# wuer5/OMGSR

Hardware: AMD Instinct MI355X
Metric: SR images/sec (higher is better)
Workload: dtype fp16; 1 GPU; OMGSR-S 256->1024, batch=4/GPU, accurate tier (fp32 stream, fp16 MFMA operands + split corrections), tiled VAE 256/64; global_batch=4, latent_tile=64, tile_overlap=32, world_size=1, parallelism=dp1, weights=seeded random, SD2.1-base shapes

## Files before the change

### omgsr_amd/build.py

```python
from __future__ import annotations

import hashlib
import os
import shutil
import subprocess
import sys

HERE = os.path.dirname(os.path.abspath(__file__))
CSRC = os.path.join(HERE, "csrc")
LIBDIR = os.path.join(HERE, "lib")
LIBNAME = "libomgsr_hip.so"
SOURCES = ["igemm.hip", "igemm_dma.hip", "igemm_p8.hip", "igemm_gmx.hip", "igemm_halo.hip", "igemm_halo_f16.hip", "igemm_halo_multi.hip", "igemm_halo_mx.hip", "igemm_halo_mx6.hip", "igemm_halo_mx6_flat.hip", "igemm_halo_out6.hip", "igemm_halo_flat.hip", "igemm_halo_gn.hip", "attention.hip", "norm.hip", "elementwise.hip", "colorfix.hip", "preprocess.hip", "mfma_peak.hip", "gemm_mxfp8.hip", "attention_mxfp8.hip"]
ARCH = "gfx950"


def lib_path() -> str:
    return os.path.join(LIBDIR, LIBNAME)


def _source_digest() -> str:
    h = hashlib.sha256()
    names = sorted(os.listdir(CSRC)) + [os.path.join("..", "..", "include", "omgsr_hip.h")]
    for n in names:
        p = os.path.join(CSRC, n)
        if os.path.isfile(p):
            h.update(n.encode())
            with open(p, "rb") as f:
                h.update(f.read())
    return h.hexdigest()


def build_library(force: bool = False, verbose: bool = False) -> str:
    hipcc = shutil.which("hipcc") or "/opt/rocm/bin/hipcc"
    os.makedirs(LIBDIR, exist_ok=True)
    out = lib_path()
    stamp = out + ".sha256"
    defs = ["-DOMGSR_BUILD_ABLATIONS"] if os.environ.get("OMGSR_BUILD_ABLATIONS", "0") == "1" else []
    defs += os.environ.get("OMGSR_EXTRA_DEFS", "").split()
    digest = _source_digest() + "".join(defs)
    if not force and os.path.isfile(out) and os.path.isfile(stamp) and open(stamp).read().strip() == digest:
        return out
    if not os.path.exists(hipcc):
        raise RuntimeError("hipcc not found: cannot build libomgsr_hip.so")
    from concurrent.futures import ThreadPoolExecutor

    hdr = hashlib.sha256()
    for n in sorted(os.listdir(CSRC)) + [os.path.join("..", "..", "include", "omgsr_hip.h")]:
        if n.endswith(".h"):
            with open(os.path.join(CSRC, n), "rb") as f:
                hdr.update(n.encode() + f.read())

    def compile_one(src: str) -> str:
        obj = os.path.join(LIBDIR, src.replace(".hip", ".o"))
        with open(os.path.join(CSRC, src), "rb") as f:
            want = hashlib.sha256(hdr.digest() + f.read() + "".join(defs).encode()).hexdigest()
        if not force and os.path.isfile(obj) and os.path.isfile(obj + ".sha256") and open(obj + ".sha256").read().strip() == want:
            return obj
        cmd = [hipcc, f"--offload-arch={ARCH}", "-O3", "-std=c++17", "-fPIC", "-Wall", "-Wno-unused-function", *defs,
               "-Rpass-analysis=kernel-resource-usage", "-c", os.path.join(CSRC, src), "-o", obj]
        if verbose:
            print(" ".join(cmd), file=sys.stderr)
        r = subprocess.run(cmd, stderr=subprocess.PIPE, text=True)
        import re
        remarks = [ln for ln in r.stderr.splitlines() if "remark:" in ln]
        rest, lines = [], r.stderr.splitlines()
        in_remark = False
        for i, ln in enumerate(lines):
            if "remark:" in ln:
                in_remark = True
                continue
            is_excerpt = bool(re.match(r"^\s*\d*\s*\|", ln)) or not ln.strip()
            if in_remark and is_excerpt:
                continue
            in_remark = False
            if ln.startswith("In file included from") and i + 1 < len(lines) and ("remark:" in lines[i + 1] or lines[i + 1].startswith("In file included")):
                continue
            if re.match(r"^\d+ (warning|remark)s? generated", ln):
                continue
            rest.append(ln)
        if rest:
            print("\n".join(rest), file=sys.stderr)
        if r.returncode != 0:
            raise subprocess.CalledProcessError(r.returncode, cmd)
        with open(os.path.join(LIBDIR, src + ".resources.txt"), "w") as f:
            f.write("\n".join(remarks) + "\n")
        with open(obj + ".sha256", "w") as f:
            f.write(want)
        return obj

    with ThreadPoolExecutor(max_workers=min(len(SOURCES), os.cpu_count() or 1)) as pool:
        objs = list(pool.map(compile_one, SOURCES))
    cmd = [hipcc, f"--offload-arch={ARCH}", "-shared", "-fPIC", "-o", out] + objs
    if verbose:
        print(" ".join(cmd), file=sys.stderr)
    subprocess.run(cmd, check=True)
    with open(stamp, "w") as f:
        f.write(digest)
    return out


def _short_name(mangled: str) -> str:
    import re
    m = re.match(r"_ZN12_GLOBAL__N_1(\d+)", mangled)
    if m:
        n = int(m.group(1))
        rest = mangled[m.end():]
        name, rest = rest[:n], rest[n:]
    else:
        m = re.match(r"_Z(\d+)", mangled)
        if not m:
            return mangled
        n = int(m.group(1))
        name, rest = mangled[m.end():m.end() + n], mangled[m.end() + n:]
    args = []
    if rest.startswith("I"):
        body = rest[1:]
        while body and not body.startswith("E"):
            for rx, fn in ((r"DF16_", lambda g: "fp16"), (r"DF16b", lambda g: "bf16"), (r"Lin(\d+)E", lambda g: "-" + g.group(1)),
                           (r"Li(\d+)E", lambda g: g.group(1)), (r"Lb([01])E", lambda g: g.group(1)), (r"f", lambda g: "float")):
                g = re.match(rx, body)
                if g:
                    args.append(fn(g))
                    body = body[g.end():]
                    break
            else:
                args.append("?")
                break
    return name + ("<" + ",".join(args) + ">" if args else "")


def kernel_resources() -> dict:
    import re
    build_library()
    keys = {"VGPRs": "vgpr", "AGPRs": "agpr", "SGPRs": "sgpr", "VGPRs Spill": "spill_vgpr", "SGPRs Spill": "spill_sgpr",
            "ScratchSize [bytes/lane]": "scratch", "Occupancy [waves/SIMD]": "occupancy", "LDS Size [bytes/block]": "lds"}
    out, mangled = {}, []
    for src in SOURCES:
        path = os.path.join(LIBDIR, src + ".resources.txt")
        if not os.path.isfile(path):
            build_library(force=True)
        cur = None
        for line in open(path):
            m = re.search(r"remark: (?:[^:]+:\d+:\d+: +)?([A-Za-z \[\]/]+): +(\S+)", line)
            if not m:
                continue
            k, v = m.group(1).strip(), m.group(2)
            if k == "Function Name":
                cur = {"source": src}
                mangled.append((v, cur))
            elif cur is not None and k in keys:
                cur[keys[k]] = int(v)
    for m, rec in mangled:
        k = _short_name(m)
        if "?" in k or k in out:
            k = m
        out[k] = rec
    return out


if __name__ == "__main__":
    print(build_library(force="--force" in sys.argv, verbose=True))
```

### omgsr_amd/csrc/igemm.hip

```cpp
#include "common.hip.h"
#include "../../include/omgsr_hip.h"
#include "timing.hip.h"
#include "igemm_epilogue.hip.h"
#include <stdlib.h>
#include <stdio.h>
#include <string.h>

namespace omgsr {
int igemm_dma_launch(const omgsr_igemm_args& a, IgemmGeo g, hipStream_t st);
int igemm_halo_launch(const omgsr_igemm_args& a, IgemmGeo g, hipStream_t st, bool phase = false);
int igemm_halo_launch_multi(const omgsr_igemm_args* a, const IgemmGeo* g0, int count, hipStream_t st, bool phase);
int igemm_halo_launch_splitk(const omgsr_igemm_args& a, const IgemmGeo& g0, int splits, hipStream_t st);
bool igemm_p8_wanted(const omgsr_igemm_args& a, const IgemmGeo& g);
int igemm_p8_launch(const omgsr_igemm_args& a, IgemmGeo g, hipStream_t st);
bool igemm_gmx_ok(const omgsr_igemm_args& a);
int igemm_gmx_launch(const omgsr_igemm_args& a, IgemmGeo g, hipStream_t st);
bool mxfp8_gemm_ok(const omgsr_igemm_args& a);
int mxfp8_gemm_launch(const omgsr_igemm_args& a, IgemmGeo g, hipStream_t st);
int igemm_halo_tiles(const omgsr_igemm_args& a, bool phase = false);
bool igemm_halo_out6_ok(const omgsr_igemm_args& a);
int igemm_halo_flat(const omgsr_igemm_args& a);
int igemm_halo_tiles_form(const omgsr_igemm_args& a, int flat);
int igemm_halo_gn_slots(const omgsr_igemm_args& a, bool phase = false);
bool igemm_halo_gn_geometry_ok(const omgsr_igemm_args& a);
}

namespace omgsr { static int g_batch_invariant = 0; }
extern "C" int omgsr_set_batch_invariant(int on) { omgsr::g_batch_invariant = (on != 0); return 0; }

namespace {

omgsr_igemm_args policy_view(const omgsr_igemm_args& a) {
    omgsr_igemm_args p = a;
    if (omgsr::g_batch_invariant && a.batch == 1) {
        const int64_t howo = (int64_t)a.Ho * a.Wo;
        const int64_t rows = a.sample_rows > 0 ? a.sample_rows : howo;
        if (rows >= howo) p.N = (int32_t)(rows / howo);
        else { p.N = 1; p.Ho = 1; p.Wo = (int32_t)rows; }
        if (p.N < 1) p.N = 1;
    }
    return p;
}

constexpr int BK = 32;
constexpr int ROWB = 80;
constexpr int NTHREADS = 256;

using Geo = IgemmGeo;

template <typename T, int BM, int BN, int WGM, int WGN>
__global__ __launch_bounds__(NTHREADS) void igemm_kernel(const omgsr_igemm_args p, const Geo g) {
    constexpr int WTM = BM / WGM, WTN = BN / WGN;
    constexpr int FM = WTM / 32, FN = WTN / 32;
    constexpr int A_CH = BM / 64, B_CH = BN / 64;
    static_assert(WGM * WGN == 4, "4 waves");
    static_assert(FM >= 1 && FN >= 1 && A_CH >= 1, "tile");
    constexpr int B_CHN = (B_CH >= 1) ? B_CH : 1;
    constexpr int STAGE_BYTES = (BM + BN) * ROWB;
    constexpr int EPI_BYTES = 4 * 32 * (WTN + 4) * 4;
    constexpr int LDS_BYTES = (2 * STAGE_BYTES > EPI_BYTES) ? 2 * STAGE_BYTES : EPI_BYTES;
    __shared__ __attribute__((aligned(16))) unsigned char lds[LDS_BYTES];

    const int t = threadIdx.x;
    const int lane = t & 63, wave = t >> 6;
    const int wm = wave / WGN, wn = wave % WGN;

    const int tile = xcd_remap(blockIdx.x, g.ntm * g.ntn);
    const int tn = tile % g.ntn, tm = tile / g.ntn;
    const int m0 = tm * BM, n0 = tn * BN;
    const int bz = blockIdx.z;

    const T* __restrict__ in = (const T*)p.in + (int64_t)bz * p.in_bstride;
    const T* __restrict__ wt = (const T*)p.weight + (int64_t)bz * p.w_bstride;

    const int kc = t & 3;
    const int r0 = t >> 2;
    int a_img[A_CH], a_vy0[A_CH], a_vx0[A_CH];
#pragma unroll
    for (int i = 0; i < A_CH; ++i) {
        const int m = m0 + r0 + 64 * i;
        if (m < g.M) {
            const int img = m / g.HoWo;
            const int rem = m - img * g.HoWo;
            const int oy = rem / p.Wo, ox = rem - oy * p.Wo;
            a_img[i] = img;
            a_vy0[i] = oy * p.stride - p.pad_top;
            a_vx0[i] = ox * p.stride - p.pad_left;
        } else {
            a_img[i] = -1; a_vy0[i] = 0; a_vx0[i] = 0;
        }
    }
    int c0 = kc * 8, tap_r = 0, tap_s = 0;
    while (c0 >= p.Cin) { c0 -= p.Cin; if (++tap_s == p.S) { tap_s = 0; ++tap_r; } }
    const int ild = p.in_ld > 0 ? p.in_ld : p.Cin;

    u32x4_t a_reg[A_CH], b_reg[B_CHN];

    auto load_stage = [&](int kt) {
        const bool tap_ok = tap_r < p.R;
#pragma unroll
        for (int i = 0; i < A_CH; ++i) {
            const int vy = a_vy0[i] + tap_r, vx = a_vx0[i] + tap_s;
            const bool ok = tap_ok && a_img[i] >= 0 && (unsigned)vy < (unsigned)g.Hv && (unsigned)vx < (unsigned)g.Wv;
            u32x4_t v = {0u, 0u, 0u, 0u};
            if (ok) {
                const int iy = vy >> p.upsample, ix = vx >> p.upsample;
                const int64_t pix = ((int64_t)a_img[i] * p.H + iy) * p.W + ix;
                v = *reinterpret_cast<const u32x4_t*>(in + pix * ild + (c0 >= ild ? c0 - ild : c0));
            }
            a_reg[i] = v;
        }
        if constexpr (B_CH >= 1) {
#pragma unroll
            for (int i = 0; i < B_CH; ++i) {
                const int n = n0 + r0 + 64 * i;
                b_reg[i] = *reinterpret_cast<const u32x4_t*>(wt + (int64_t)n * p.K_pad + kt * BK + kc * 8);
            }
        } else {
            if (r0 < BN) b_reg[0] = *reinterpret_cast<const u32x4_t*>(wt + (int64_t)(n0 + r0) * p.K_pad + kt * BK + kc * 8);
        }
        c0 += BK;
        while (c0 >= p.Cin) { c0 -= p.Cin; if (++tap_s == p.S) { tap_s = 0; ++tap_r; } }
    };
    auto write_stage = [&](int buf) {
        unsigned char* As = lds + buf * STAGE_BYTES;
        unsigned char* Bs = As + BM * ROWB;
#pragma unroll
        for (int i = 0; i < A_CH; ++i)
            *reinterpret_cast<u32x4_t*>(As + (r0 + 64 * i) * ROWB + kc * 16) = a_reg[i];
        if constexpr (B_CH >= 1) {
#pragma unroll
            for (int i = 0; i < B_CH; ++i)
                *reinterpret_cast<u32x4_t*>(Bs + (r0 + 64 * i) * ROWB + kc * 16) = b_reg[i];
        } else {
            if (r0 < BN) *reinterpret_cast<u32x4_t*>(Bs + r0 * ROWB + kc * 16) = b_reg[0];
        }
    };

    f32x16_t acc[FM][FN];
#pragma unroll
    for (int i = 0; i < FM; ++i)
#pragma unroll
        for (int j = 0; j < FN; ++j)
#pragma unroll
            for (int r = 0; r < 16; ++r) acc[i][j][r] = 0.0f;

    load_stage(0);
    write_stage(0);
    __syncthreads();

    const int frag_off = (lane & 31) * ROWB + (lane >> 5) * 16;
    for (int kt = 0; kt < g.nk; ++kt) {
        const int buf = kt & 1;
        if (kt + 1 < g.nk) load_stage(kt + 1);
        const unsigned char* As = lds + buf * STAGE_BYTES + wm * WTM * ROWB + frag_off;
        const unsigned char* Bs = lds + buf * STAGE_BYTES + BM * ROWB + wn * WTN * ROWB + frag_off;
#pragma unroll
        for (int ks = 0; ks < 2; ++ks) {
            x8_t<T> af[FM], bf[FN];
#pragma unroll
            for (int i = 0; i < FM; ++i) af[i] = *reinterpret_cast<const x8_t<T>*>(As + i * 32 * ROWB + ks * 32);
#pragma unroll
            for (int j = 0; j < FN; ++j) bf[j] = *reinterpret_cast<const x8_t<T>*>(Bs + j * 32 * ROWB + ks * 32);
#pragma unroll
            for (int i = 0; i < FM; ++i)
#pragma unroll
                for (int j = 0; j < FN; ++j) acc[i][j] = mfma32(bf[j], af[i], acc[i][j]);
        }
        if (kt + 1 < g.nk) write_stage(buf ^ 1);
        __syncthreads();
    }

    float* epi = reinterpret_cast<float*>(lds) + wave * 32 * (WTN + 4);
    igemm_epilogue_linear<T, WTN, FM, FN>(p, g.M, acc, epi, lane, m0 + wm * WTM, n0 + wn * WTN, bz, p.gn_partial ? g.HoWo : 0);
}

template <int BM, int BN, int WGM, int WGN>
int launch(const omgsr_igemm_args& a, Geo g, hipStream_t st) {
    g.ntm = (g.M + BM - 1) / BM;
    const int logical_cols = (a.act == OMGSR_ACT_GEGLU) ? 2 * a.Cout : a.Cout;
    g.ntn = (logical_cols + BN - 1) / BN;
    dim3 grid(g.ntm * g.ntn, 1, a.batch);
    OMGSR_DISPATCH_T(hipLaunchKernelGGL((igemm_kernel<T, BM, BN, WGM, WGN>), grid, dim3(NTHREADS), 0, st, a, g));
    return (int)hipGetLastError();
}

template <typename T>
__global__ __launch_bounds__(256) void splitk_reduce_kernel(const omgsr_igemm_args p, const float* __restrict__ ws, const int M,
                                                            const int ldw, const int splits) {
    const bool geglu = (p.act == OMGSR_ACT_GEGLU);
    const int oct_per_row = (p.Cout + 7) >> 3;
    const int64_t i = (int64_t)blockIdx.x * blockDim.x + threadIdx.x;
    if (i >= (int64_t)M * oct_per_row) return;
    const int m = (int)(i / oct_per_row), n = (int)(i - (int64_t)m * oct_per_row) * 8;
    float v[8];
    if (geglu) {
        const int pc = (n >> 5) * 64 + (n & 31);
        float a[8], gt[8];
#pragma unroll
        for (int e = 0; e < 8; ++e) { a[e] = 0.0f; gt[e] = 0.0f; }
        for (int sidx = 0; sidx < splits; ++sidx) {
            const float* r = ws + ((int64_t)sidx * M + m) * ldw + pc;
#pragma unroll
            for (int e = 0; e < 8; ++e) { a[e] += r[e]; gt[e] += r[32 + e]; }
        }
#pragma unroll
        for (int e = 0; e < 8; ++e) {
            float x = a[e] * p.alpha, y = gt[e] * p.alpha;
            if (p.bias) { x += p.bias[pc + e]; y += p.bias[pc + 32 + e]; }
            v[e] = x * gelu_erf_f(y);
        }
    } else {
#pragma unroll
        for (int e = 0; e < 8; ++e) v[e] = 0.0f;
        for (int sidx = 0; sidx < splits; ++sidx) {
            const f32x4_t* r = reinterpret_cast<const f32x4_t*>(ws + ((int64_t)sidx * M + m) * ldw + n);
            const f32x4_t r0 = r[0], r1 = r[1];
#pragma unroll
            for (int e = 0; e < 4; ++e) { v[e] += r0[e]; v[4 + e] += r1[e]; }
        }
#pragma unroll
        for (int e = 0; e < 8; ++e) {
            float x = v[e] * p.alpha;
            if (p.bias && n + e < p.Cout) x += p.bias[n + e];
            if (p.act == OMGSR_ACT_SILU) x = silu_f(x);
            else if (p.act == OMGSR_ACT_GELU_TANH) x = gelu_tanh_f(x);
            v[e] = x;
        }
    }
    const int64_t ldo = p.out_ld > 0 ? p.out_ld : p.Cout;
    float amax = 0.0f;
    if constexpr (std::is_same<T, f16_t>::value) {
        if (p.out_mx) {
#pragma unroll
            for (int e = 0; e < 8; ++e) {
                float x = v[e];
                if (p.gate) x *= p.gate[n + e];
                if (p.residual) x += p.res_el == OMGSR_EL_F32 ? ((const float*)p.residual)[(int64_t)m * p.Cout + n + e]
                                                               : (float)((const T*)p.residual)[(int64_t)m * p.Cout + n + e];
                v[e] = x;
                amax = fmaxf(amax, fabsf(x));
            }
            if (p.out_mx == 6) store8_mx6<T>(p.out, (int64_t)m * 4 * p.Cout, p.Cout, n, v);
            else store8_mx<T>(p.out, (int64_t)m * 4 * p.Cout, p.Cout, n, v);
            if (p.overflow_flag && amax > 65504.0f) atomicOr(p.overflow_flag, 1u);
            if (p.overflow_flag && p.out_mx == 1 && amax > 448.0f) atomicOr(p.overflow_flag, 2u);
            return;
        }
    }
    if ((p.Cout & 7) == 0 && (ldo & 7) == 0 && (p.out_lo_off & 7) == 0) {
        if (p.gate) {
#pragma unroll
            for (int e = 0; e < 8; ++e) v[e] *= p.gate[n + e];
        }
        if (p.residual) {
            float rf[8];
            if (p.res_el == OMGSR_EL_F32) load8<T, true>(p.residual, (int64_t)m * p.Cout + n, rf);
            else load8<T, false>(p.residual, (int64_t)m * p.Cout + n, rf);
#pragma unroll
            for (int e = 0; e < 8; ++e) v[e] += rf[e];
        }
        const int64_t o = (int64_t)m * ldo + n;
        if (p.out_dtype == OMGSR_OUT_BF16) {
#pragma unroll
            for (int e = 0; e < 8; ++e) amax = fmaxf(amax, fabsf(v[e]));
            if (p.out_lo_off > 0) store8<T, 2>(p.out, o, p.out_lo_off, v);
            else store8<T, 0>(p.out, o, 0, v);
            if constexpr (std::is_same<T, f16_t>::value) {
                if (p.overflow_flag && amax > 65504.0f) atomicOr(p.overflow_flag, 1u);
            }
        } else store8<T, 1>(p.out, o, 0, v);
        return;
    }
    for (int e = 0; e < 8 && n + e < p.Cout; ++e) {
        float x = v[e];
        if (p.gate) x *= p.gate[n + e];
        if (p.residual) x += p.res_el == OMGSR_EL_F32 ? ((const float*)p.residual)[(int64_t)m * p.Cout + n + e]
                                                       : (float)((const T*)p.residual)[(int64_t)m * p.Cout + n + e];
        if (p.out_dtype == OMGSR_OUT_BF16) {
            amax = fmaxf(amax, fabsf(x));
            if constexpr (std::is_same<T, f16_t>::value) x = __builtin_amdgcn_fmed3f(x, -65504.0f, 65504.0f);
            const T hi = (T)x;
            ((T*)p.out)[(int64_t)m * ldo + n + e] = hi;
            if (p.out_lo_off > 0) ((T*)p.out)[(int64_t)m * ldo + p.out_lo_off + n + e] = (T)(x - (float)hi);
        } else ((float*)p.out)[(int64_t)m * ldo + n + e] = x;
    }
    if constexpr (std::is_same<T, f16_t>::value) {
        if (p.overflow_flag && p.out_dtype == OMGSR_OUT_BF16 && amax > 65504.0f) atomicOr(p.overflow_flag, 1u);
    }
}

bool use_halo(const omgsr_igemm_args& a);
bool use_halo_phase(const omgsr_igemm_args& a);
bool out_mx6_ok(const omgsr_igemm_args& a);
int halo_splitk_plan(const omgsr_igemm_args& a);

int halo_splitk_plan(const omgsr_igemm_args& a) {
    static const char* off = getenv("OMGSR_HALO_SPLITK");
    if (off && off[0] == '0') return 1;
    const int logical_cols = (a.act == OMGSR_ACT_GEGLU) ? 2 * a.Cout : a.Cout;
    if (a.in_ld != 0 || a.gn_scale_shift || a.out_layout != OMGSR_LAYOUT_NHWC || a.act == OMGSR_ACT_GEGLU || logical_cols < 96 || a.upsample ||
        a.group_tiles != 0 || a.batch != 1) return 1;
    if (a.mx_chunks16 <= 0 || omgsr::igemm_halo_flat(a) != 0) return 1;
    const int tiles = omgsr::igemm_halo_tiles(a);
    static const char* mt = getenv("OMGSR_HALO_SPLITK_MAX_TILES");
    static const int max_tiles = mt ? atoi(mt) : 128;
    if (tiles <= 0 || tiles >= max_tiles) return 1;
    const int nk = a.Cin / 32;
    const bool mx = a.mx_chunks16 > 0;
    static const char* tg = getenv("OMGSR_HALO_SPLITK_TARGET");
    static const int target = tg ? atoi(tg) : 512;
    int splits = target / tiles;
    if (splits > 8) splits = 8;
    if (mx) {
        splits &= ~1;
        const int n16 = a.mx_chunks16, n8 = nk - n16;
        while (splits >= 2 && (n16 / (splits / 2) < 2 || n8 / (splits / 2) < 2)) splits -= 2;
    } else {
        while (splits >= 2 && nk / splits < 2) --splits;
    }
    return splits < 2 ? 1 : splits;
}

int splitk_plan(const omgsr_igemm_args& a_real, int64_t M64) {
    const omgsr_igemm_args a = policy_view(a_real);
    if (omgsr::g_batch_invariant) M64 = (int64_t)a.N * a.Ho * a.Wo;
    const int logical_cols = (a.act == OMGSR_ACT_GEGLU) ? 2 * a.Cout : a.Cout;
    if (use_halo_phase(a)) return 1;
    if (use_halo(a)) return halo_splitk_plan(a);
    if (a.batch != 1 || a.out_layout != OMGSR_LAYOUT_NHWC || (a.Cin % 32) || (a.in_ld % 32) || logical_cols < 96 || a.mx_chunks16 > 0) return 1;
    if (a.out_mx && a.act == OMGSR_ACT_GEGLU) return 1;
    const int nk = a.K_pad / 32;
    const int64_t tiles = ((M64 + 255) / 256) * ((logical_cols + 127) / 128);
    const int slots = 512;
    if (tiles >= slots / 2 || nk < 48) return 1;
    int splits = (int)(slots / tiles);
    if (splits > 8) splits = 8;
    while (splits > 1 && nk / splits < 16) --splits;
    return splits < 2 ? 1 : splits;
}

bool mx_geometry_ok(const omgsr_igemm_args& a) {
    const int logical_cols = (a.act == OMGSR_ACT_GEGLU) ? 2 * a.Cout : a.Cout;
    const bool common = a.R == 3 && a.S == 3 && a.stride == 1 && a.pad_top == 1 && a.pad_left == 1 && (a.Cin % 128) == 0 && a.in_ld == 0 && a.batch == 1 &&
                        logical_cols >= 96 && a.act != OMGSR_ACT_GEGLU && a.out_layout == OMGSR_LAYOUT_NHWC && a.mx_chunks16 == a.Cin / 64 &&
                        omgsr::compute_dtype() == 1;
    if (a.upsample) return common && a.weight_ph && a.Ho == 2 * a.H && a.Wo == 2 * a.W && (a.Cout & 7) == 0 && !a.residual;
    return common && a.weight_cm && a.Ho == a.H && a.Wo == a.W;
}

bool use_halo(const omgsr_igemm_args& a_real) {
    if (a_real.mx_chunks16 > 0) return !a_real.upsample && mx_geometry_ok(a_real);
    const omgsr_igemm_args a = policy_view(a_real);
    static const char* mode = getenv("OMGSR_IGEMM_MODE");
    const int logical_cols = (a.act == OMGSR_ACT_GEGLU) ? 2 * a.Cout : a.Cout;
    const bool halo_ok = a.weight_cm && a.R == 3 && a.S == 3 && a.stride == 1 && a.pad_top == 1 && a.pad_left == 1 &&
                         (a.Cin % 32) == 0 && (a.in_ld % 32) == 0 && a.batch == 1 && a.Ho == (a.H << a.upsample) && a.Wo == (a.W << a.upsample) && a.Wo >= 16 &&
                         (logical_cols >= 96 || (logical_cols <= 32 && a.act != OMGSR_ACT_GEGLU)) &&
                         a.out_layout == OMGSR_LAYOUT_NHWC;
    if (!halo_ok || (mode && (!strcmp(mode, "reg") || !strcmp(mode, "dma")))) return false;
    if (mode && !strcmp(mode, "halo")) return true;
    const int padded_w = ((a.Wo + 31) / 32) * 32;
    if (padded_w * 3 > a.Wo * 4 && !omgsr::igemm_halo_flat(a)) return false;
    const int tiles = omgsr::igemm_halo_tiles(a);
    const int gt = a.group_tiles < 0 ? -a.group_tiles : a.group_tiles;
    return (tiles > gt ? tiles : gt) >= 192;
}

bool out_mx6_ok(const omgsr_igemm_args& a) {
    if (a.upsample || a.act == OMGSR_ACT_GEGLU || a.out_dtype != OMGSR_OUT_BF16 || a.out_layout != OMGSR_LAYOUT_NHWC) return false;
    return omgsr::igemm_halo_out6_ok(a) && use_halo(a);
}

bool use_halo_phase(const omgsr_igemm_args& a_real) {
    if (a_real.mx_chunks16 > 0) return a_real.upsample && mx_geometry_ok(a_real);
    const omgsr_igemm_args a = policy_view(a_real);
    static const char* off = getenv("OMGSR_UPSAMPLE_PHASES");
    static const char* mode = getenv("OMGSR_IGEMM_MODE");
    if ((off && off[0] == '0') || (mode && (!strcmp(mode, "reg") || !strcmp(mode, "dma")))) return false;
    const bool ok = a.weight_ph && a.upsample == 1 && a.R == 3 && a.S == 3 && a.stride == 1 && a.pad_top == 1 && a.pad_left == 1 &&
                    (a.Cin % 32) == 0 && (a.in_ld % 32) == 0 && a.batch == 1 && a.Ho == 2 * a.H && a.Wo == 2 * a.W && a.W >= 16 &&
                    a.Cout >= 96 && (a.Cout & 7) == 0 && a.act != OMGSR_ACT_GEGLU && a.out_layout == OMGSR_LAYOUT_NHWC && !a.residual;
    if (!ok) return false;
    const int padded_w = ((a.W + 31) / 32) * 32;
    if (padded_w * 3 > a.W * 4) return false;
    const int tiles = omgsr::igemm_halo_tiles(a, true);
    const int gt = a.group_tiles < 0 ? -a.group_tiles : a.group_tiles;
    return (tiles > gt ? tiles : gt) >= 192;
}

}

namespace {
void gn_plan(const omgsr_igemm_args& a, int* nslot, int* entries) {
    *nslot = 0; *entries = 0;
    if (a.gn_groups <= 0 || a.Cout <= 0 || (a.Cout % a.gn_groups)) return;
    const int gsz = a.Cout / a.gn_groups;
    const bool pow2 = gsz == 4 || gsz == 8 || gsz == 16 || gsz == 32 || gsz == 64;
    const int64_t ldo = a.out_ld > 0 ? a.out_ld : a.Cout;
    if ((a.Cout & 7) || (ldo & 7) || a.act == OMGSR_ACT_GEGLU || a.out_layout != OMGSR_LAYOUT_NHWC || a.batch != 1) return;
    const int64_t M64 = (int64_t)a.N * a.Ho * a.Wo;
    if (use_halo_phase(a)) {
        *nslot = omgsr::igemm_halo_gn_slots(a, true);
        *entries = pow2 ? a.gn_groups : a.Cout;
        return;
    }
    if (use_halo(a)) {
        if (a.Cout < 96) return;
        *nslot = omgsr::igemm_halo_gn_slots(a);
        *entries = pow2 ? a.gn_groups : a.Cout;
        return;
    }
    if (a.workspace && splitk_plan(a, M64) > 1) return;
    if (omgsr::g_batch_invariant) return;
    const int howo = a.Ho * a.Wo;
    if (howo % 32) return;
    *nslot = howo / 32;
    *entries = (pow2 && gsz <= 32) ? a.gn_groups : a.Cout;
}
}

namespace {
bool gn_fusable(const omgsr_igemm_args& a_in) {
    static const char* off = getenv("OMGSR_GN_FUSE");
    if (off && off[0] == '0') return false;
    omgsr_igemm_args a = a_in;
    a.gn_scale_shift = nullptr;
    if (!omgsr::igemm_halo_gn_geometry_ok(a) || a.out_layout != OMGSR_LAYOUT_NHWC || a.act == OMGSR_ACT_GEGLU) return false;
    if ((int64_t)a.H * a.W * a.Cin >= (1ll << 31)) return false;
    if (a.workspace && splitk_plan(a, (int64_t)a.N * a.Ho * a.Wo) > 1) return false;
    if (!use_halo(a) || use_halo_phase(a)) return false;
    if (omgsr::igemm_halo_flat(a) != 0) return false;
    static const char* mc = getenv("OMGSR_GN_FUSE_MAX_COUT");
    static const int max_cout = mc ? atoi(mc) : 128;
    const int logical_cols = (a.act == OMGSR_ACT_GEGLU) ? 2 * a.Cout : a.Cout;
    return logical_cols <= max_cout;
}
}

extern "C" int32_t omgsr_igemm_gn_fusable(const omgsr_igemm_args* ap) { return (ap && gn_fusable(*ap)) ? 1 : 0; }
extern "C" int32_t omgsr_igemm_out_mx6_ok(const omgsr_igemm_args* ap) {
    if (!ap) return 0;
    omgsr_igemm_args a = *ap;
    a.out_mx = 6;
    return out_mx6_ok(a) ? 1 : 0;
}

extern "C" int32_t omgsr_igemm_gn_slots(const omgsr_igemm_args* ap) {
    if (!ap) return 0;
    int nslot, entries;
    gn_plan(*ap, &nslot, &entries);
    return nslot;
}

extern "C" int32_t omgsr_igemm_gn_entries(const omgsr_igemm_args* ap) {
    if (!ap) return 0;
    int nslot, entries;
    gn_plan(*ap, &nslot, &entries);
    return entries;
}

extern "C" int64_t omgsr_igemm_workspace_bytes(const omgsr_igemm_args* ap) {
    if (!ap || ap->mxf8) return 0;
    const int64_t M64 = (int64_t)ap->N * ap->Ho * ap->Wo;
    const int splits = splitk_plan(*ap, M64);
    if (splits < 2) return 0;
    const int logical_cols = (ap->act == OMGSR_ACT_GEGLU) ? 2 * ap->Cout : ap->Cout;
    return (int64_t)splits * M64 * (((logical_cols + 127) / 128) * 128) * 4;
}

namespace {
int validate_args(omgsr_igemm_args& a) {
    if (!a.in || !a.weight || !a.out) return OMGSR_E_BADARG;
    if (a.N <= 0 || a.H <= 0 || a.W <= 0 || a.Cin <= 0 || a.Cout <= 0 || a.Ho <= 0 || a.Wo <= 0 ||
        a.R <= 0 || a.S <= 0 || a.stride <= 0 || a.batch <= 0) return OMGSR_E_BADARG;
    if ((a.Cin & 7) || (a.Cout_pad & 127) || (a.K_pad % BK) || a.K_pad < a.R * a.S * a.Cin) return OMGSR_E_SHAPE;
    if (a.upsample != 0 && a.upsample != 1) return OMGSR_E_BADARG;
    const int64_t M64 = (int64_t)a.N * a.Ho * a.Wo;
    if (M64 >= (1ll << 31)) return OMGSR_E_SHAPE;
    const int logical_cols = (a.act == OMGSR_ACT_GEGLU) ? 2 * a.Cout : a.Cout;
    if (logical_cols > a.Cout_pad) return OMGSR_E_SHAPE;
    if (a.act == OMGSR_ACT_GEGLU && ((a.Cout & 31) || a.out_layout != OMGSR_LAYOUT_NHWC)) return OMGSR_E_SHAPE;
    if (a.out_layout == OMGSR_LAYOUT_T && (a.t_rows <= 0 || a.t_ld < a.t_rows || a.residual)) return OMGSR_E_BADARG;
    if (a.out_ld != 0 && (a.out_ld < a.Cout || a.out_layout != OMGSR_LAYOUT_NHWC)) return OMGSR_E_BADARG;
    if (a.res_el != OMGSR_EL_16 && a.res_el != OMGSR_EL_F32) return OMGSR_E_BADARG;
    if (a.res_el == OMGSR_EL_F32 && a.residual && a.act == OMGSR_ACT_GEGLU) return OMGSR_E_SHAPE;
    if (a.out_lo_off < 0) return OMGSR_E_BADARG;
    if (a.out_lo_off && (a.out_dtype != OMGSR_OUT_BF16 || a.out_layout != OMGSR_LAYOUT_NHWC || (a.Cout & 7) || (a.out_ld & 7) || (a.out_lo_off & 7) ||
                         a.out_lo_off < a.Cout || a.out_ld < a.out_lo_off + a.Cout || a.gn_partial)) return OMGSR_E_SHAPE;
    if (a.in_split && ((a.in_ld > 0 ? a.in_ld : a.Cin) & 15)) return OMGSR_E_SHAPE;
    if (a.in_ld < 0 || (a.in_ld & 7) || (a.in_ld > 0 && (a.in_ld > a.Cin || a.Cin > 2 * a.in_ld))) return OMGSR_E_SHAPE;
    if (a.in_ld == a.Cin) a.in_ld = 0;
    const int ksegs = 1 + (a.in_split ? 1 : 0) + (a.w_split ? 1 : 0);
    if (a.Cin % (8 * ksegs)) return OMGSR_E_SHAPE;
    if (a.mx_chunks16 < 0 || (a.mx_chunks16 > 0 && !mx_geometry_ok(a) && !omgsr::igemm_gmx_ok(a))) return OMGSR_E_SHAPE;
    if (a.mx_chunks16 > 0 && a.mx_fmt != 0 && a.mx_fmt != 8 && (a.mx_fmt != 6 || !mx_geometry_ok(a))) return OMGSR_E_SHAPE;
    if (a.out_mx != 0 && a.out_mx != 1 && a.out_mx != 6) return OMGSR_E_BADARG;
    if (a.out_mx == 6 && !out_mx6_ok(a)) return OMGSR_E_SHAPE;
    if (a.out_mx && (a.out_dtype != OMGSR_OUT_BF16 || a.out_layout != OMGSR_LAYOUT_NHWC || (a.Cout & 63) || a.out_lo_off || a.out_ld || a.gn_partial ||
                     omgsr::compute_dtype() != 1)) return OMGSR_E_SHAPE;
    if (a.gn_scale_shift && (a.gn_nimg <= 0 || a.gn_act != OMGSR_ACT_SILU || !gn_fusable(a))) return OMGSR_E_SHAPE;
    if (a.mxf8 != 0 && a.mxf8 != 1) return OMGSR_E_BADARG;
    if (a.mxf8 && !omgsr::mxfp8_gemm_ok(a)) return OMGSR_E_SHAPE;
    if (a.gn_partial) {
        int nslot, entries;
        gn_plan(a, &nslot, &entries);
        if (nslot <= 0 || a.gn_entries != entries) return OMGSR_E_BADARG;
    }
    return 0;
}

void work_of(const omgsr_igemm_args& a, double* flops, double* bytes) {
    const int64_t M64 = (int64_t)a.N * a.Ho * a.Wo;
    const int logical_cols = (a.act == OMGSR_ACT_GEGLU) ? 2 * a.Cout : a.Cout;
    const int ksegs = 1 + (a.in_split ? 1 : 0) + (a.w_split ? 1 : 0);
    *flops = 2.0 * (double)M64 * (double)a.R * a.S * (a.Cin / ksegs) * (double)logical_cols * a.batch;
    const double out_b = (a.out_dtype == OMGSR_OUT_F32 ? 4.0 : (a.out_lo_off ? 4.0 : 2.0)), res_b = a.residual ? (a.res_el == OMGSR_EL_F32 ? 4.0 : 2.0) : 0.0;
    const double eb = a.mxf8 ? 1.0 + 1.0 / 32.0 : 2.0;
    *bytes = (eb * ((double)a.N * a.H * a.W * (a.in_ld > 0 ? a.in_ld : a.Cin) + (double)a.Cout_pad * a.K_pad) + (double)M64 * a.Cout * (out_b + res_b)) * a.batch;
}

Geo geo_of(const omgsr_igemm_args& a) {
    Geo g{};
    g.M = (int)((int64_t)a.N * a.Ho * a.Wo);
    g.HoWo = a.Ho * a.Wo;
    g.Hv = a.H << a.upsample;
    g.Wv = a.W << a.upsample;
    g.nk = a.K_pad / BK;
    g.splits = 1; g.nk_total = g.nk;
    return g;
}
}

extern "C" int omgsr_igemm_multi_plan(omgsr_igemm_args* args, int32_t count) {
    if (!args || count <= 0) return OMGSR_E_BADARG;
    static const char* off = getenv("OMGSR_MULTI");
    int total = 0, total_ph = 0, total_flat = 0;
    bool all_flat_ok = true;
    for (int i = 0; i < count; ++i) {
        args[i].group_tiles = 0;
        total += omgsr::igemm_halo_tiles_form(args[i], 0);
        total_ph += omgsr::igemm_halo_tiles(args[i], true);
        const int tf = omgsr::igemm_halo_tiles_form(args[i], 1);
        all_flat_ok = all_flat_ok && tf > 0;
        total_flat += tf > 0 ? tf : 0;
    }
    if ((off && off[0] == '0') || omgsr::g_batch_invariant) return 0;
    const bool flat = all_flat_ok && total_flat < total;
    for (int i = 0; i < count; ++i) args[i].group_tiles = (args[i].upsample && args[i].weight_ph) ? total_ph : (flat ? -total_flat : total);
    return 0;
}

extern "C" int omgsr_igemm_multi(const omgsr_igemm_args* args, int32_t count, void* stream) {
    if (!args || count <= 0) return OMGSR_E_BADARG;
    hipStream_t st = (hipStream_t)stream;
    constexpr int MAXG = 8;
    omgsr_igemm_args grp[MAXG];
    Geo geo[MAXG];
    int ng = 0, mode = -1;
    double gf = 0.0, gb = 0.0;
    long long gm = 0;
    auto flush = [&]() -> int {
        if (ng == 0) return 0;
        int rc;
        {
            const int logical_cols = (grp[0].act == OMGSR_ACT_GEGLU) ? 2 * grp[0].Cout : grp[0].Cout;
            omgsr::TimingScope ts(OMGSR_TK_IGEMM, gf, gb, st, gm, logical_cols, (long long)grp[0].R * grp[0].S * grp[0].Cin);
            ts.rec.variant = ng == 1 ? (mode == 1 ? 6 : 3) : (mode == 1 ? 8 : 7);
            if (grp[0].gn_scale_shift) ts.rec.variant = ng == 1 ? 10 : 11;
            if (grp[0].mx_chunks16 > 0 && grp[0].mx_fmt == 6) ts.rec.variant = mode == 1 ? (ng == 1 ? 16 : 17) : (ng == 1 ? 13 : 14);
            rc = ng == 1 ? omgsr::igemm_halo_launch(grp[0], geo[0], st, mode == 1) : omgsr::igemm_halo_launch_multi(grp, geo, ng, st, mode == 1);
        }
        ng = 0; gf = gb = 0.0; gm = 0;
        return rc;
    };
    for (int i = 0; i < count; ++i) {
        omgsr_igemm_args a = args[i];
        int rc = validate_args(a);
        if (rc != 0) { flush(); return rc; }
        const int m = (a.workspace && splitk_plan(a, (int64_t)a.N * a.Ho * a.Wo) > 1) ? -1 : use_halo_phase(a) ? 1 : use_halo(a) ? 0 : -1;
        const bool same = ng > 0 && m == mode && a.weight == grp[0].weight && a.Cin == grp[0].Cin && a.in_ld == grp[0].in_ld && a.Cout == grp[0].Cout &&
                          a.act == grp[0].act && a.out_dtype == grp[0].out_dtype && a.out_lo_off == grp[0].out_lo_off && a.out_ld == grp[0].out_ld &&
                          a.res_el == grp[0].res_el && (a.residual != nullptr) == (grp[0].residual != nullptr) &&
                          (a.gn_partial != nullptr) == (grp[0].gn_partial != nullptr) && a.gn_entries == grp[0].gn_entries && a.bias == grp[0].bias &&
                          a.gate == grp[0].gate && a.alpha == grp[0].alpha && a.upsample == grp[0].upsample && a.mx_chunks16 == grp[0].mx_chunks16 && a.mx_fmt == grp[0].mx_fmt && a.out_mx == grp[0].out_mx &&
                          ((a.Cout <= 32) == (grp[0].Cout <= 32)) && ((omgsr::igemm_halo_flat(a) != 0) == (omgsr::igemm_halo_flat(grp[0]) != 0)) &&
                          (a.gn_scale_shift != nullptr) == (grp[0].gn_scale_shift != nullptr) && a.gn_act == grp[0].gn_act;
        if (m < 0) {
            rc = flush();
            if (rc == 0) rc = omgsr_igemm(&args[i], stream);
            if (rc != 0) return rc;
            continue;
        }
        if (ng > 0 && (!same || ng == MAXG)) { rc = flush(); if (rc != 0) return rc; }
        mode = m;
        double f, b;
        work_of(a, &f, &b);
        gf += f; gb += b; gm += (long long)a.N * a.Ho * a.Wo;
        geo[ng] = geo_of(a);
        grp[ng++] = a;
    }
    return flush();
}

extern "C" int omgsr_igemm(const omgsr_igemm_args* ap, void* stream) {
    if (!ap) return OMGSR_E_BADARG;
    omgsr_igemm_args a = *ap;
    {
        const int rc = validate_args(a);
        if (rc != 0) return rc;
    }
    const int64_t M64 = (int64_t)a.N * a.Ho * a.Wo;
    const int logical_cols = (a.act == OMGSR_ACT_GEGLU) ? 2 * a.Cout : a.Cout;
    Geo g{};
    g.M = (int)M64;
    g.HoWo = a.Ho * a.Wo;
    g.Hv = a.H << a.upsample;
    g.Wv = a.W << a.upsample;
    g.nk = a.K_pad / BK;
    hipStream_t st = (hipStream_t)stream;
    double flops, bytes;
    work_of(a, &flops, &bytes);
    omgsr::TimingScope ts(OMGSR_TK_IGEMM, flops, bytes, st, M64 * a.batch, logical_cols, (long long)a.R * a.S * a.Cin);
    const omgsr_igemm_args pv = policy_view(a);
    const int64_t Mp = omgsr::g_batch_invariant ? (int64_t)pv.N * pv.Ho * pv.Wo : M64;
    const int64_t pbatch = omgsr::g_batch_invariant ? 1 : a.batch;
    if (a.mxf8) {
        ts.rec.variant = 18;
        return omgsr::mxfp8_gemm_launch(a, g, st);
    }
    const int64_t tiles128 = ((Mp + 127) / 128) * (a.Cout_pad / 128) * pbatch;
    static const char* mode = getenv("OMGSR_IGEMM_MODE");
    const int64_t tiles256 = ((Mp + 255) / 256) * ((logical_cols + 127) / 128) * pbatch;
    g.splits = 1; g.nk_total = g.nk;
    if (a.workspace && !(mode && (!strcmp(mode, "reg") || !strcmp(mode, "halo")))) {
        const int splits = splitk_plan(a, M64);
        if (splits > 1) {
            if (a.gn_partial) return OMGSR_E_BADARG;
            int rc;
            if (use_halo(a)) {
                ts.rec.variant = a.mx_fmt == 6 ? 15 : 12;
                rc = omgsr::igemm_halo_launch_splitk(a, g, splits, st);
            } else {
                g.splits = splits;
                ts.rec.variant = 4;
                rc = omgsr::igemm_dma_launch(a, g, st);
            }
            if (rc != 0) return rc;
            const int ldw = ((logical_cols + 127) / 128) * 128;
            const int64_t items = M64 * ((a.Cout + 7) / 8);
            OMGSR_DISPATCH_T(hipLaunchKernelGGL(splitk_reduce_kernel<T>, dim3((unsigned)((items + 255) / 256)), dim3(256), 0, st, a,
                                                (const float*)a.workspace, (int)M64, ldw, splits));
            return (int)hipGetLastError();
        }
    }
    if (a.mx_chunks16 > 0 && omgsr::igemm_gmx_ok(a)) {
        static const char* pm = getenv("OMGSR_P8_MX");
        if (!(pm && pm[0] == '0') && !omgsr::g_batch_invariant && a.batch == 1 && omgsr::igemm_p8_wanted(a, g)) {
            ts.rec.variant = 5;
            return omgsr::igemm_p8_launch(a, g, st);
        }
        ts.rec.variant = 9;
        return omgsr::igemm_gmx_launch(a, g, st);
    }
    if (use_halo_phase(a)) { ts.rec.variant = (a.mx_chunks16 > 0 && a.mx_fmt == 6) ? 16 : 6; return omgsr::igemm_halo_launch(a, g, st, true); }
    if (use_halo(a)) { ts.rec.variant = a.gn_scale_shift ? 10 : (a.mx_chunks16 > 0 && a.mx_fmt == 6) ? 13 : 3; return omgsr::igemm_halo_launch(a, g, st); }
    if (a.gn_scale_shift) return OMGSR_E_SHAPE;
    {
        static const char* dbg = getenv("OMGSR_DEBUG_DISPATCH");
        if (dbg && a.R == 3)
            fprintf(stderr, "[omgsr] 3x3 off the halo path: N %d H %d W %d Cin %d Cout %d stride %d pad %d,%d ups %d Ho %d Wo %d cm %d batch %d act %d layout %d tiles %d\n",
                    a.N, a.H, a.W, a.Cin, a.Cout, a.stride, a.pad_top, a.pad_left, a.upsample, a.Ho, a.Wo, a.weight_cm != nullptr, a.batch, a.act, a.out_layout,
                    omgsr::igemm_halo_tiles(a));
    }
    const bool dma_ok = logical_cols >= 96 && (a.Cin % 32) == 0 && (a.in_ld % 32) == 0;
    static const char* dsm = getenv("OMGSR_DMA_SMALL");
    const bool gemm_shaped = a.R == 1 && a.S == 1 && a.stride == 1 && a.pad_top == 0 && a.pad_left == 0 && !a.upsample && a.Ho == a.H && a.Wo == a.W;
    const bool dma_small = !(dsm && dsm[0] == '0') && gemm_shaped && a.batch == 1 && a.K_pad >= 256 && a.out_layout == OMGSR_LAYOUT_NHWC && Mp >= 64;
    if (dma_ok && ((mode && !strcmp(mode, "dma")) || (!(mode && !strcmp(mode, "reg")) && (tiles256 >= 192 || dma_small)))) {
        static const char* p8 = getenv("OMGSR_P8");
        if (!(p8 && p8[0] == '0') && !omgsr::g_batch_invariant && omgsr::igemm_p8_wanted(a, g)) {
            ts.rec.variant = 5;
            return omgsr::igemm_p8_launch(a, g, st);
        }
        ts.rec.variant = 2;
        return omgsr::igemm_dma_launch(a, g, st);
    }
    ts.rec.variant = 1;
    if (a.act == OMGSR_ACT_GEGLU) return launch<128, 128, 2, 2>(a, g, st);
    if (logical_cols <= 32) return launch<128, 32, 4, 1>(a, g, st);
    if (logical_cols <= 64 || tiles128 < 192) return launch<64, 64, 2, 2>(a, g, st);
    return launch<128, 128, 2, 2>(a, g, st);
}
```

Before: 20.82 images/s.

## Add thin-output 3x3 conv kernel treating taps as GEMM columns

Adds a dedicated kernel for 3x3 stride-1 convolutions with at most 8 output channels and many input channels. It folds the 9 taps times Cout into the GEMM N dimension, computes per-pixel partial products over a haloed region with MFMA, stages them in LDS, and sums the shifted taps in the epilogue. The aim is to avoid wasting the wide-N tiles of the halo igemm path on a tiny Cout. The cost is extra halo rows and columns of compute plus a large LDS buffer, and it bypasses grouped launches for these convs.

```diff
diff --git a/omgsr_amd/build.py b/omgsr_amd/build.py
--- a/omgsr_amd/build.py
+++ b/omgsr_amd/build.py
@@ -10,7 +10,7 @@
 CSRC = os.path.join(HERE, "csrc")
 LIBDIR = os.path.join(HERE, "lib")
 LIBNAME = "libomgsr_hip.so"
-SOURCES = ["igemm.hip", "igemm_dma.hip", "igemm_p8.hip", "igemm_gmx.hip", "igemm_halo.hip", "igemm_halo_f16.hip", "igemm_halo_multi.hip", "igemm_halo_mx.hip", "igemm_halo_mx6.hip", "igemm_halo_mx6_flat.hip", "igemm_halo_out6.hip", "igemm_halo_flat.hip", "igemm_halo_gn.hip", "attention.hip", "norm.hip", "elementwise.hip", "colorfix.hip", "preprocess.hip", "mfma_peak.hip", "gemm_mxfp8.hip", "attention_mxfp8.hip"]
+SOURCES = ["igemm.hip", "igemm_dma.hip", "igemm_p8.hip", "igemm_gmx.hip", "igemm_halo.hip", "igemm_halo_f16.hip", "igemm_halo_multi.hip", "igemm_halo_mx.hip", "igemm_halo_mx6.hip", "igemm_halo_mx6_flat.hip", "igemm_halo_out6.hip", "igemm_halo_flat.hip", "igemm_halo_gn.hip", "conv_thin.hip", "attention.hip", "norm.hip", "elementwise.hip", "colorfix.hip", "preprocess.hip", "mfma_peak.hip", "gemm_mxfp8.hip", "attention_mxfp8.hip"]
 ARCH = "gfx950"
 
 
diff --git a/omgsr_amd/csrc/conv_thin.hip b/omgsr_amd/csrc/conv_thin.hip
--- /dev/null
+++ b/omgsr_amd/csrc/conv_thin.hip
@@ -0,0 +1,199 @@
+#include "common.hip.h"
+#include "../../include/omgsr_hip.h"
+#include "igemm_epilogue.hip.h"
+
+namespace omgsr {
+namespace {
+
+constexpr int TN_RH = 8, TN_RW = 32;
+constexpr int TN_OH = TN_RH - 2, TN_OW = TN_RW - 2;
+constexpr int TN_FM = TN_RH * TN_RW / 16 / 4;
+constexpr int TN_NF = 5;
+constexpr int TN_PST = 72;
+constexpr int TN_LDS = TN_RH * TN_RW * TN_PST * 4;
+static_assert(TN_FM * 16 * 4 == TN_RH * TN_RW, "region = whole fragments, 4 waves");
+
+OMGSR_DEVINL f32x4_t mfma16(bf16x8_t a, bf16x8_t b, f32x4_t c) { return __builtin_amdgcn_mfma_f32_16x16x32_bf16(a, b, c, 0, 0, 0); }
+OMGSR_DEVINL f32x4_t mfma16(f16x8_t a, f16x8_t b, f32x4_t c) { return __builtin_amdgcn_mfma_f32_16x16x32_f16(a, b, c, 0, 0, 0); }
+
+template <typename T>
+OMGSR_DEVINL void thin_epilogue8(const omgsr_igemm_args& p, const int64_t m, float (&v)[8]) {
+#pragma unroll
+    for (int e = 0; e < 8; ++e) {
+        float x = v[e] * p.alpha;
+        if (p.bias && e < p.Cout) x += p.bias[e];
+        if (p.act == OMGSR_ACT_SILU) x = silu_f(x);
+        else if (p.act == OMGSR_ACT_GELU_TANH) x = gelu_tanh_f(x);
+        v[e] = x;
+    }
+    const int64_t ldo = p.out_ld > 0 ? p.out_ld : p.Cout;
+    float amax = 0.0f;
+    if (p.Cout == 8 && (ldo & 7) == 0 && (p.out_lo_off & 7) == 0) {
+        if (p.gate) {
+#pragma unroll
+            for (int e = 0; e < 8; ++e) v[e] *= p.gate[e];
+        }
+        if (p.residual) {
+            float rf[8];
+            if (p.res_el == OMGSR_EL_F32) load8<T, true>(p.residual, m * 8, rf);
+            else load8<T, false>(p.residual, m * 8, rf);
+#pragma unroll
+            for (int e = 0; e < 8; ++e) v[e] += rf[e];
+        }
+        const int64_t o = m * ldo;
+        if (p.out_dtype == OMGSR_OUT_BF16) {
+#pragma unroll
+            for (int e = 0; e < 8; ++e) amax = fmaxf(amax, fabsf(v[e]));
+            if (p.out_lo_off > 0) store8<T, 2>(p.out, o, p.out_lo_off, v);
+            else store8<T, 0>(p.out, o, 0, v);
+            if constexpr (std::is_same<T, f16_t>::value) {
+                if (p.overflow_flag && amax > 65504.0f) atomicOr(p.overflow_flag, 1u);
+            }
+        } else store8<T, 1>(p.out, o, 0, v);
+        return;
+    }
+    for (int e = 0; e < 8 && e < p.Cout; ++e) {
+        float x = v[e];
+        if (p.gate) x *= p.gate[e];
+        if (p.residual) x += p.res_el == OMGSR_EL_F32 ? ((const float*)p.residual)[m * p.Cout + e] : (float)((const T*)p.residual)[m * p.Cout + e];
+        if (p.out_dtype == OMGSR_OUT_BF16) {
+            amax = fmaxf(amax, fabsf(x));
+            if constexpr (std::is_same<T, f16_t>::value) x = __builtin_amdgcn_fmed3f(x, -65504.0f, 65504.0f);
+            const T hi = (T)x;
+            ((T*)p.out)[m * ldo + e] = hi;
+            if (p.out_lo_off > 0) ((T*)p.out)[m * ldo + p.out_lo_off + e] = (T)(x - (float)hi);
+        } else ((float*)p.out)[m * ldo + e] = x;
+    }
+    if constexpr (std::is_same<T, f16_t>::value) {
+        if (p.overflow_flag && p.out_dtype == OMGSR_OUT_BF16 && amax > 65504.0f) atomicOr(p.overflow_flag, 1u);
+    }
+}
+
+template <typename T>
+__global__ __launch_bounds__(256, 2) void conv_thin_n_kernel(const omgsr_igemm_args p, const int tiles_x, const int tiles_y) {
+    extern __shared__ __attribute__((aligned(16))) float P[];
+    const int t = threadIdx.x, lane = t & 63, wave = t >> 6;
+    const int per_img = tiles_x * tiles_y;
+    const int tile = xcd_remap(blockIdx.x, gridDim.x);
+    const int img = tile / per_img, rt = tile - img * per_img;
+    const int ty = rt / tiles_x, tx = rt - ty * tiles_x;
+    const int oy0 = ty * TN_OH, ox0 = tx * TN_OW;
+    const int ild = p.in_ld > 0 ? p.in_ld : p.Cin;
+    const T* __restrict__ in = (const T*)p.in;
+    const T* __restrict__ wt = (const T*)p.weight;
+    const int kq = lane >> 4;
+
+    int64_t a_off[TN_FM];
+#pragma unroll
+    for (int f = 0; f < TN_FM; ++f) {
+        const int q = (wave * TN_FM + f) * 16 + (lane & 15);
+        const int iy = oy0 - 1 + q / TN_RW, ix = ox0 - 1 + q % TN_RW;
+        a_off[f] = ((unsigned)iy < (unsigned)p.H && (unsigned)ix < (unsigned)p.W) ? (((int64_t)img * p.H + iy) * p.W + ix) * ild : -1;
+    }
+    int64_t b_off[TN_NF];
+#pragma unroll
+    for (int j = 0; j < TN_NF; ++j) {
+        const int n = j * 16 + (lane & 15);
+        const int tap = n / p.Cout, co = n - tap * p.Cout;
+        b_off[j] = tap < 9 ? (int64_t)co * p.K_pad + tap * p.Cin : -1;
+    }
+
+    const u32x4_t zero = {0u, 0u, 0u, 0u};
+    auto load = [&](const int ks, u32x4_t (&a)[TN_FM], u32x4_t (&b)[TN_NF]) {
+        const int c = ks * 32 + kq * 8;
+        const bool cok = c < p.Cin;
+        const int ph = c >= ild ? c - ild : c;
+#pragma unroll
+        for (int f = 0; f < TN_FM; ++f) a[f] = (cok && a_off[f] >= 0) ? *reinterpret_cast<const u32x4_t*>(in + a_off[f] + ph) : zero;
+#pragma unroll
+        for (int j = 0; j < TN_NF; ++j) b[j] = (cok && b_off[j] >= 0) ? *reinterpret_cast<const u32x4_t*>(wt + b_off[j] + c) : zero;
+    };
+
+    f32x4_t acc[TN_FM][TN_NF];
+#pragma unroll
+    for (int f = 0; f < TN_FM; ++f)
+#pragma unroll
+        for (int j = 0; j < TN_NF; ++j) acc[f][j] = f32x4_t{0.0f, 0.0f, 0.0f, 0.0f};
+
+    const int nks = (p.Cin + 31) / 32;
+    u32x4_t a0[TN_FM], b0[TN_NF], a1[TN_FM], b1[TN_NF];
+    load(0, a0, b0);
+    for (int ks = 0; ks < nks; ++ks) {
+        if (ks + 1 < nks) load(ks + 1, a1, b1);
+#pragma unroll
+        for (int f = 0; f < TN_FM; ++f)
+#pragma unroll
+            for (int j = 0; j < TN_NF; ++j)
+                acc[f][j] = mfma16(__builtin_bit_cast(x8_t<T>, a0[f]), __builtin_bit_cast(x8_t<T>, b0[j]), acc[f][j]);
+#pragma unroll
+        for (int f = 0; f < TN_FM; ++f) a0[f] = a1[f];
+#pragma unroll
+        for (int j = 0; j < TN_NF; ++j) b0[j] = b1[j];
+    }
+
+#pragma unroll
+    for (int f = 0; f < TN_FM; ++f)
+#pragma unroll
+        for (int j = 0; j < TN_NF; ++j) {
+            const int n = j * 16 + (lane & 15);
+            if (j < TN_NF - 1 || n < TN_PST) {
+#pragma unroll
+                for (int i = 0; i < 4; ++i) P[((wave * TN_FM + f) * 16 + 4 * kq + i) * TN_PST + n] = acc[f][j][i];
+            }
+        }
+    __syncthreads();
+
+    if (t >= TN_OH * TN_OW) return;
+    const int oy = t / TN_OW, ox = t - oy * TN_OW;
+    const int y = oy0 + oy, x = ox0 + ox;
+    if (y >= p.Ho || x >= p.Wo) return;
+    float v[8];
+#pragma unroll
+    for (int e = 0; e < 8; ++e) v[e] = 0.0f;
+    if (p.Cout == 8) {
+#pragma unroll
+        for (int tap = 0; tap < 9; ++tap) {
+            const float* src = P + ((oy + tap / 3) * TN_RW + ox + tap % 3) * TN_PST + tap * 8;
+            const f32x4_t s0 = *reinterpret_cast<const f32x4_t*>(src), s1 = *reinterpret_cast<const f32x4_t*>(src + 4);
+#pragma unroll
+            for (int e = 0; e < 4; ++e) { v[e] += s0[e]; v[4 + e] += s1[e]; }
+        }
+    } else {
+#pragma unroll
+        for (int tap = 0; tap < 9; ++tap) {
+            const float* src = P + ((oy + tap / 3) * TN_RW + ox + tap % 3) * TN_PST + tap * p.Cout;
+#pragma unroll
+            for (int e = 0; e < 8; ++e)
+                if (e < p.Cout) v[e] += src[e];
+        }
+    }
+    thin_epilogue8<T>(p, ((int64_t)img * p.Ho + y) * p.Wo + x, v);
+}
+
+}
+
+bool conv_thin_n_ok(const omgsr_igemm_args& a) {
+    return a.R == 3 && a.S == 3 && a.stride == 1 && a.pad_top == 1 && a.pad_left == 1 && !a.upsample && a.Ho == a.H && a.Wo == a.W &&
+           a.Cout >= 1 && a.Cout <= 8 && a.act != OMGSR_ACT_GEGLU && a.out_layout == OMGSR_LAYOUT_NHWC && a.batch == 1 && a.mx_chunks16 == 0 &&
+           a.mxf8 == 0 && a.out_mx == 0 && a.gn_partial == nullptr && a.gn_scale_shift == nullptr && (a.Cin % 8) == 0 &&
+           (int64_t)a.N * a.H * a.W < (1ll << 31);
+}
+
+int conv_thin_n_launch(const omgsr_igemm_args& a, hipStream_t st) {
+    static bool attr_set = false;
+    if (!attr_set) {
+        const void* fns[] = {reinterpret_cast<const void*>(conv_thin_n_kernel<bf16_t>), reinterpret_cast<const void*>(conv_thin_n_kernel<f16_t>)};
+        for (const void* f : fns) {
+            const hipError_t e = hipFuncSetAttribute(f, hipFuncAttributeMaxDynamicSharedMemorySize, TN_LDS);
+            if (e != hipSuccess) return (int)e;
+        }
+        attr_set = true;
+    }
+    const int tiles_x = (a.Wo + TN_OW - 1) / TN_OW, tiles_y = (a.Ho + TN_OH - 1) / TN_OH;
+    const int64_t blocks = (int64_t)tiles_x * tiles_y * a.N;
+    if (blocks >= (1ll << 31)) return OMGSR_E_SHAPE;
+    OMGSR_DISPATCH_T(hipLaunchKernelGGL(conv_thin_n_kernel<T>, dim3((unsigned)blocks), dim3(256), TN_LDS, st, a, tiles_x, tiles_y));
+    return (int)hipGetLastError();
+}
+
+}
diff --git a/omgsr_amd/csrc/igemm.hip b/omgsr_amd/csrc/igemm.hip
--- a/omgsr_amd/csrc/igemm.hip
+++ b/omgsr_amd/csrc/igemm.hip
@@ -23,6 +23,9 @@
 int igemm_halo_tiles_form(const omgsr_igemm_args& a, int flat);
 int igemm_halo_gn_slots(const omgsr_igemm_args& a, bool phase = false);
 bool igemm_halo_gn_geometry_ok(const omgsr_igemm_args& a);
+bool conv_thin_n_ok(const omgsr_igemm_args& a);
+int conv_thin_n_launch(const omgsr_igemm_args& a, hipStream_t st);
+constexpr int kVariantThinN = 19;
 }
 
 namespace omgsr { static int g_batch_invariant = 0; }
@@ -387,6 +390,13 @@
     const int tiles = omgsr::igemm_halo_tiles(a, true);
     const int gt = a.group_tiles < 0 ? -a.group_tiles : a.group_tiles;
     return (tiles > gt ? tiles : gt) >= 192;
+}
+
+bool use_thin_n(const omgsr_igemm_args& a) {
+    static const char* off = getenv("OMGSR_THIN_N");
+    static const char* mode = getenv("OMGSR_IGEMM_MODE");
+    if ((off && off[0] == '0') || mode) return false;
+    return a.gn_groups <= 0 && omgsr::conv_thin_n_ok(a) && (int64_t)a.Ho * a.Wo >= 1024 && a.Cin >= 512;
 }
 
 }
@@ -578,7 +588,7 @@
         omgsr_igemm_args a = args[i];
         int rc = validate_args(a);
         if (rc != 0) { flush(); return rc; }
-        const int m = (a.workspace && splitk_plan(a, (int64_t)a.N * a.Ho * a.Wo) > 1) ? -1 : use_halo_phase(a) ? 1 : use_halo(a) ? 0 : -1;
+        const int m = (a.workspace && splitk_plan(a, (int64_t)a.N * a.Ho * a.Wo) > 1) || use_thin_n(a) ? -1 : use_halo_phase(a) ? 1 : use_halo(a) ? 0 : -1;
         const bool same = ng > 0 && m == mode && a.weight == grp[0].weight && a.Cin == grp[0].Cin && a.in_ld == grp[0].in_ld && a.Cout == grp[0].Cout &&
                           a.act == grp[0].act && a.out_dtype == grp[0].out_dtype && a.out_lo_off == grp[0].out_lo_off && a.out_ld == grp[0].out_ld &&
                           a.res_el == grp[0].res_el && (a.residual != nullptr) == (grp[0].residual != nullptr) &&
@@ -663,6 +673,7 @@
         ts.rec.variant = 9;
         return omgsr::igemm_gmx_launch(a, g, st);
     }
+    if (use_thin_n(a)) { ts.rec.variant = omgsr::kVariantThinN; return omgsr::conv_thin_n_launch(a, st); }
     if (use_halo_phase(a)) { ts.rec.variant = (a.mx_chunks16 > 0 && a.mx_fmt == 6) ? 16 : 6; return omgsr::igemm_halo_launch(a, g, st, true); }
     if (use_halo(a)) { ts.rec.variant = a.gn_scale_shift ? 10 : (a.mx_chunks16 > 0 && a.mx_fmt == 6) ? 13 : 3; return omgsr::igemm_halo_launch(a, g, st); }
     if (a.gn_scale_shift) return OMGSR_E_SHAPE;
```

After: 20.88 images/s (median of 6 runs). No clear change (+0.3%).
